# paramhanji/sin-inn

Hardware: AMD Instinct MI355X
Metric: training frames/sec at 256x256 bs=16 (higher is better)
Workload: dtype f32; 1 GPU; BASELINE configs[1]: 8-block INN (SRF, -c 4 x 2 levels), 256x256x3, fp32, synthetic clip (64 frames, lr_window 10), batch 16/GPU, full training step (fwd+bwd, rev+bwd, Adam); height=256, width=256, global_batch=16, num_coupling=4, architecture=SRF, parallelism=dp1, hip_graph=False

## Files before the change

### include/sininn.h

```cpp
#ifndef SININN_H
#define SININN_H

#include <stddef.h>
#include <stdint.h>

#ifdef __cplusplus
extern "C" {
#endif

#define SININN_ABI_VERSION 4
#define SININN_HIDDEN 256

int sininn_version(void);
const char* sininn_last_error(void);
size_t sininn_sizeof(int which);
int sininn_stream_priority_range(int* least, int* greatest);
int sininn_stream_create(int priority, void** stream);
int sininn_capture_unjoined(void* origin, void** streams, int n, int* flags);

int sininn_pack_conv_weights(const float* w_oihw, const float* bias, int N, int Cin, int ksize,
                             const int* colmap, int Np, float* w_fwd, float* b_fwd,
                             int Cdp, float* w_dgrad, void* stream);

int sininn_pack_conv_weights_bf16(const float* w_oihw, const float* bias, int N, int Cin, int ksize,
// ... 65 lines not shown
int sininn_conv_sub1_fwd(const sininn_conv_args* first, const sininn_conv_args* second, void* stream);

size_t sininn_conv_sub1_bwd_workspace_bytes(int cin, int co);
int sininn_conv_sub1_bwd(const sininn_conv_args* recompute, const sininn_conv_args* d2, const sininn_conv_args* d1, int no_dx,
                         float* gw2, float* gb2, float* gw1, float* gb1, void* workspace, size_t workspace_bytes, void* stream);

size_t sininn_conv_sub1_wide_bwd_workspace_bytes(int cin, int co);
int sininn_conv_sub1_wide_bwd(const sininn_conv_args* d2, const sininn_conv_args* d1, const float* x, int x_stride, float* gw1, float* gb1,
                              void* workspace, size_t workspace_bytes, void* stream);
size_t sininn_conv_sub1_wide_wg2_workspace_bytes(int cin, int co);
int sininn_conv_sub1_wide_wg2(const float* dr, int dr_stride, const void* h, int h_stride, int B, int H, int W, float* gw2, float* gb2,
                              void* workspace, size_t workspace_bytes, void* stream);

int sininn_conv3_smallk_bits_supported(const sininn_conv_args* args);
int sininn_conv3_smallk_bits(const sininn_conv_args* args, unsigned* bits, void* stream);

int sininn_conv_sub3_supported(const sininn_conv_args* first, const sininn_conv_args* second);
int sininn_conv_sub3(const sininn_conv_args* first, const sininn_conv_args* second, void* stream);

size_t sininn_wgrad_workspace_bytes(int N, int Cin, int ksize, int B, int H, int W);
int sininn_wgrad(const float* in, int in_stride, int Cin, const float* dout, int dout_stride, int N,
                 int B, int H, int W, int ksize, float* gw_oihw, float* gbias,
                 void* workspace, size_t workspace_bytes, void* stream);

typedef struct sininn_wgrad_item {
  size_t struct_bytes;
  const float* in;   int in_stride;   int Cin;
  const float* dout; int dout_stride; int N;
  float* gw; float* gb;
  int in_bf16, dout_bf16;
  int in_group_stride, dout_group_stride;
  int gap_begin, gap_len;
} sininn_wgrad_item;
size_t sininn_wgrad_group_workspace_bytes(const sininn_wgrad_item* items, int n, int B, int H, int W, int ksize);
int sininn_wgrad_group(const sininn_wgrad_item* items, int n, int B, int H, int W, int ksize,
                       void* workspace, size_t workspace_bytes, void* stream);

int sininn_coupling_bwd(const float* dy, int dy_stride, const int* dy_map,
                        const float* vy, int vy_stride, const int* vy_map,
                        const float* s, const float* gld, int B, int HW, int Co, float clamp,
                        int inverse, float* dr, float* dv, int dv_stride, void* stream);

int sininn_haar(const float* in, const int64_t in_strides[4], float* out, const int64_t out_strides[4],
                int B, int C, int H, int W, int inverse, void* stream);
int sininn_lrelu_bwd(float* g, int g_stride, const float* f, int f_stride, int64_t M, int n, float slope, void* stream);
int sininn_irn_tail(const float* v, int v_stride, const float* h, const float* g, int64_t M, int Co, float clamp, int inverse,
// ... 281 lines not shown
```

### sin-inn_amd/_lib.py

```python
import ctypes as C
import os

_HERE = os.path.dirname(os.path.abspath(__file__))
LIB_PATH = os.environ.get('SININN_LIB', os.path.join(_HERE, 'libsininn.so'))

c_f = C.c_void_p
c_i = C.c_void_p
I64x4 = C.c_int64 * 4


class ConvArgs(C.Structure):
    _fields_ = [
        ('inp', c_f), ('in_stride', C.c_int), ('Cin', C.c_int),
        ('w', c_f), ('bias', c_f), ('Np', C.c_int), ('winograd', C.c_int),
        ('B', C.c_int), ('H', C.c_int), ('W', C.c_int), ('ksize', C.c_int),
        ('mode', C.c_int),
        ('out', c_f), ('out_stride', C.c_int), ('N', C.c_int),
        ('out_map', c_i),
        ('v', c_f), ('v_stride', C.c_int),
        ('out2', c_f), ('out2_stride', C.c_int),
        ('sbuf', c_f),
        ('logdet', c_f),
        ('Co', C.c_int), ('clamp', C.c_float), ('col_tile', C.c_int),
        ('mask', c_f), ('mask_stride', C.c_int),
# ... 149 lines not shown
                                               C.c_void_p, C.c_void_p]),
    'sininn_pack_winograd': (C.c_int, [c_f, C.c_int, C.c_int, c_i, C.c_int, c_f, C.c_int, c_f, C.c_void_p]),
    'sininn_pack_work_items': (C.c_int, [C.POINTER(PackDesc)]),
    'sininn_pack_batch': (C.c_int, [C.c_void_p, C.c_int, C.c_int, C.c_void_p]),
    'sininn_softsplat': (C.c_int, [c_f, c_f, C.c_int, C.c_int, C.c_int, C.c_int, c_f, C.c_void_p]),
    'sininn_softsplat_bwd': (C.c_int, [c_f, c_f, c_f, C.c_int, C.c_int, C.c_int, C.c_int, c_f, c_f, C.c_void_p]),
    'sininn_occlusion_wang': (C.c_int, [c_f, C.c_int, C.c_int, C.c_int, C.c_float, c_f, c_f, C.c_void_p]),
    'sininn_census': (C.c_int, [c_f, c_f, c_f, C.c_int, C.c_int, C.c_int, C.c_int, C.c_int, C.c_float, c_f, c_f, C.c_void_p]),
    'sininn_census_bwd': (C.c_int, [c_f, c_f, c_f, C.c_int, C.c_int, C.c_int, C.c_int, C.c_int, C.c_float, c_f, c_f, c_f, c_f, C.c_void_p]),
    'sininn_masked_l1': (C.c_int, [c_f, c_f, c_f, C.c_int, C.c_int, C.c_int, C.c_int, C.c_int, C.c_float, c_f, c_f, C.c_void_p]),
    'sininn_masked_l1_bwd': (C.c_int, [c_f, c_f, c_f, C.c_int, C.c_int, C.c_int, C.c_int, C.c_int, C.c_float, c_f, c_f, c_f, c_f, C.c_void_p]),
    'sininn_occlusion_brox': (C.c_int, [c_f, c_f, C.c_int, C.c_int, C.c_int, C.c_void_p, C.c_void_p]),
    'sininn_ssim': (C.c_int, [c_f, c_f, c_f, C.c_int, C.c_int, C.c_int, C.c_int, C.c_int, C.c_int, C.c_float, c_f, c_f, C.c_void_p]),
    'sininn_ssim_bwd': (C.c_int, [c_f, c_f, c_f, C.c_int, C.c_int, C.c_int, C.c_int, C.c_int, C.c_int, C.c_float, c_f, c_f, c_f, c_f, C.c_void_p]),
    'sininn_bilateral_smooth': (C.c_int, [c_f, c_f, C.c_int, C.c_int, C.c_int, C.c_int, C.c_int, C.c_int, C.c_float, C.c_float, c_f, c_f, C.c_void_p]),
    'sininn_bilateral_smooth_bwd': (C.c_int, [c_f, c_f, C.c_int, C.c_int, C.c_int, C.c_int, C.c_int, C.c_int, C.c_float, C.c_float, c_f, c_f, C.c_void_p]),
    'sininn_coupling_colmap': (None, [C.c_int, C.c_int, C.POINTER(C.c_int)]),
    'sininn_conv': (C.c_int, [C.POINTER(ConvArgs), C.c_void_p]),
    'sininn_conv_test_hooks': (None, [C.c_int, C.c_int]),
    'sininn_wgrad_test_hooks': (None, [C.c_int]),
    'sininn_pair_k1_test_hook': (None, [C.c_int]),
    'sininn_sub1_bwd_test_hook': (None, [C.c_int]),
    'sininn_wgrad_workspace_bytes': (C.c_size_t, [C.c_int] * 6),
    'sininn_wgrad': (C.c_int, [c_f, C.c_int, C.c_int, c_f, C.c_int, C.c_int, C.c_int, C.c_int, C.c_int, C.c_int,
                               c_f, c_f, C.c_void_p, C.c_size_t, C.c_void_p]),
    'sininn_wgrad_group_workspace_bytes': (C.c_size_t, [C.POINTER(WgradItem), C.c_int, C.c_int, C.c_int, C.c_int, C.c_int]),
    'sininn_wgrad_group': (C.c_int, [C.POINTER(WgradItem), C.c_int, C.c_int, C.c_int, C.c_int, C.c_int, C.c_void_p,
                                     C.c_size_t, C.c_void_p]),
    'sininn_coupling_bwd': (C.c_int, [c_f, C.c_int, c_i, c_f, C.c_int, c_i, c_f, c_f, C.c_int, C.c_int, C.c_int,
                                      C.c_float, C.c_int, c_f, c_f, C.c_int, C.c_void_p]),
    'sininn_profile_begin': (None, [C.c_int, C.c_void_p, C.c_int]),
    'sininn_wall_clock_khz': (C.c_int, []),
    'sininn_profile_end': (C.c_int, [C.POINTER(C.c_int), C.POINTER(C.c_float)]),
    'sininn_profile_classes_begin': (None, []),
    'sininn_profile_classes_end': (C.c_int, [C.c_int, C.POINTER(C.c_double), C.POINTER(C.c_double), C.POINTER(C.c_int)]),
    'sininn_profile_classes_bytes': (C.c_int, [C.c_int, C.POINTER(C.c_double)]),
    'sininn_glow_saved_floats': (C.c_size_t, [C.c_int] * 4),
    'sininn_glow_saved_floats_dtype': (C.c_size_t, [C.c_int] * 5),
    'sininn_glow_scratch_bytes': (C.c_size_t, [C.c_int] * 5),
    'sininn_glow_scratch_bytes_dtype': (C.c_size_t, [C.c_int] * 6),
    'sininn_glow_forward': (C.c_int, [C.POINTER(GlowArgs), C.c_void_p]),
    'sininn_glow_backward': (C.c_int, [C.POINTER(GlowArgs), C.c_void_p, C.c_void_p]),
    'sininn_glow_hidden_gates': (C.c_int, [C.POINTER(GlowArgs), C.c_int, C.c_void_p, C.c_void_p]),
    'sininn_glow_group_major_fits': (C.c_int, [C.c_int, C.c_int, C.c_int]),
    'sininn_capture_unjoined': (C.c_int, [C.c_void_p, C.POINTER(C.c_void_p), C.c_int, C.POINTER(C.c_int)]),
    'sininn_conv_pair_k1_supported': (C.c_int, [C.POINTER(ConvArgs), C.POINTER(ConvArgs)]),
# ... 124 lines not shown
```

### sin-inn_amd/csrc/api.cpp

```cpp
#include <stdarg.h>
#include <string.h>

#include <unordered_map>
#include <unordered_set>
#include <vector>

#include "common.h"

namespace sininn {

static thread_local char g_err[512] = "";
void set_error(const char* fmt, ...) {
  va_list ap;
  va_start(ap, fmt);
  vsnprintf(g_err, sizeof(g_err), fmt, ap);
  va_end(ap);
}

int conv_launch(const sininn_conv_args* a, hipStream_t st);
int conv_pair_k1_supported(const sininn_conv_args* f, const sininn_conv_args* s);
size_t conv_sub1_bwd_workspace_bytes(int cond_cin, int co);
int conv_sub1_bwd_launch(const sininn_conv_args* rc, const sininn_conv_args* d2, const sininn_conv_args* d1, int no_dx, void* ws,
                         size_t ws_bytes, int* slabs_out, hipStream_t st);
int conv_sub1_bwd_reduce(int cond_cin, int co, const void* ws, int slabs, float* gw2, float* gb2, float* gw1, float* gb1, hipStream_t st);
void conv_sub1_bwd_enable(int on);
void conv3_smallk_enable(int on);
size_t conv_sub1_bf16_wide_ws_bytes(int ksize, int dtype, int cond_cin, int co);
int conv_sub1_bf16_wide_bwd_supported(const sininn_conv_args* d2, const sininn_conv_args* d1);
int conv_sub1_bf16_wide_bwd_launch(const sininn_conv_args* d2, const sininn_conv_args* d1, hipStream_t st);
int conv_sub1_bf16_wide_bwd_wg1_launch(const sininn_conv_args* d2, const sininn_conv_args* d1, const float* x, int x_stride, void* ws, size_t ws_bytes,
                                       int* slabs_out, hipStream_t st);
int conv_sub1_bf16_wide_reduce(const void* ws, int slabs, float* gw1, float* gb1, hipStream_t st);
size_t conv_sub1_bf16_wide_wg2_ws_bytes(int ksize, int dtype, int cond_cin, int co);
int conv_sub1_bf16_wide_wg2_launch(const float* dr, int dr_stride, const void* h, int h_stride, int B, int H, int W, void* ws, size_t ws_bytes,
                                   float* gw2, float* gb2, hipStream_t st);
int conv3_smallk_bf16_supported(const sininn_conv_args* a);
int conv3_smallk_bf16_launch_bits(const sininn_conv_args* a, unsigned* bits, hipStream_t st);
int conv_sub1_fwd_supported(const sininn_conv_args* f, const sininn_conv_args* s);
int conv_sub1_fwd_launch(const sininn_conv_args* f, const sininn_conv_args* s, hipStream_t st);
int conv_pair_k1_launch(const sininn_conv_args* f, const sininn_conv_args* s, hipStream_t st);
void conv_pair_k1_enable(int on);
int conv_sub3_bf16_supported(const sininn_conv_args* f, const sininn_conv_args* s);
int conv_sub3_bf16_launch(const sininn_conv_args* f, const sininn_conv_args* s, hipStream_t st);
void sub3_fusion_set(int on);
void conv_set_test_hooks(int force_cfg, int force_ck);
void wgrad_set_force16(int on);
size_t wgrad_workspace_bytes(int N, int Cin, int ksize, int B, int H, int W);
int wgrad_launch(const float* in, int in_stride, int Cin, const float* dout, int dout_stride, int N, int B, int H, int W,
                 int ksize, float* gw, float* gb, void* ws, size_t ws_bytes, hipStream_t st);
size_t wgrad_group_workspace_bytes(const sininn_wgrad_item* items, int n, int B, int H, int W, int ksize);
int wgrad_group_launch(const sininn_wgrad_item* items, int n, int B, int H, int W, int ksize, void* ws, size_t ws_bytes,
                       hipStream_t st);
int pack_launch(const float* w, const float* bias, int N, int Cin, int ksize, const int* colmap, int Np, float* w_fwd,
                float* b_fwd, int Cdp, float* w_dgrad, hipStream_t st);
int coupling_bwd_launch(const float* dy, int dy_stride, const int* dy_map, const float* vy, int vy_stride,
                        const int* vy_map, const float* s, const float* gld, int B, int HW, int Co, float clamp,
                        int inverse, float* dr, float* dv, int dv_stride, hipStream_t st);
int squeeze_launch(const float* in, const int64_t is[4], float* out, const int64_t os[4], int B, int C, int H, int W,
                   int levels, int inverse, const int* chan_map, int map_on_out, hipStream_t st);
int permute_launch(const float* in, int in_stride, float* out, int out_stride, int64_t M, int C, const int* idx,
                   hipStream_t st);
int sqdiff_sum_launch(const float* x, const int64_t xs[4], const float* y, const int64_t ys[4], int B, int C, int H,
                      int W, float* out, hipStream_t st);
int sqdiff_bwd_launch(const float* x, const int64_t xs[4], const float* y, const int64_t ys[4], int B, int C, int H,
                      int W, const float* scale, float gscale, float* gx, const int64_t gxs[4], float* gy,
                      const int64_t gys[4], hipStream_t st);
int mmd_gram_launch(const float* x, const int64_t xs[4], const float* y, const int64_t ys[4], int B, int C, int H,
                    int W, float* g, hipStream_t st);
int mmd_finish_launch(const float* g, int B, int rev, float* out, float* coef, hipStream_t st);
// ... 304 lines not shown
    SININN_CHECK(!gw1 && !gb1, "sininn_conv_sub1_wide_bwd: gw1 / gb1 need x");
    return conv_sub1_bf16_wide_bwd_launch(d2, d1, ST(stream));
  }
  int slabs = 0;
  if (int rc = conv_sub1_bf16_wide_bwd_wg1_launch(d2, d1, x, x_stride, workspace, workspace_bytes, &slabs, ST(stream))) return rc;
  if (!gw1 && !gb1) return 0;
  return conv_sub1_bf16_wide_reduce(workspace, slabs, gw1, gb1, ST(stream));
}
size_t sininn_conv_sub1_wide_wg2_workspace_bytes(int cin, int co) { return conv_sub1_bf16_wide_wg2_ws_bytes(1, 1, cin, co); }
int sininn_conv_sub1_wide_wg2(const float* dr, int dr_stride, const void* h, int h_stride, int B, int H, int W, float* gw2, float* gb2,
                              void* workspace, size_t workspace_bytes, void* stream) {
  SININN_CHECK(sininn_conv_sub1_wide_wg2_workspace_bytes(96, 96) > 0, "sininn_conv_sub1_wide_wg2: the wide kernels are switched off");
  return conv_sub1_bf16_wide_wg2_launch(dr, dr_stride, h, h_stride, B, H, W, workspace, workspace_bytes, gw2, gb2, ST(stream));
}
int sininn_conv3_smallk_bits_supported(const sininn_conv_args* args) { return conv3_smallk_bf16_supported(args); }
int sininn_conv3_smallk_bits(const sininn_conv_args* args, unsigned* bits, void* stream) {
  SININN_CHECK(bits != nullptr, "sininn_conv3_smallk_bits: bits is NULL");
  return conv3_smallk_bf16_launch_bits(args, bits, ST(stream));
}
void sininn_sub1_bwd_test_hook(int on) { conv_sub1_bwd_enable(on); conv3_smallk_enable(on); }

void sininn_conv_test_hooks(int force_cfg, int force_ck) { conv_set_test_hooks(force_cfg, force_ck); }
void sininn_wgrad_test_hooks(int force16) { wgrad_set_force16(force16); }
void sininn_pair_k1_test_hook(int on) { conv_pair_k1_enable(on & 1); sub3_fusion_set((on & 4) ? 1 : ((on & 2) ? 0 : -1)); }
int sininn_conv_sub3_supported(const sininn_conv_args* first, const sininn_conv_args* second) {
  return conv_sub3_bf16_supported(first, second);
}
int sininn_conv_sub3(const sininn_conv_args* first, const sininn_conv_args* second, void* stream) {
  return conv_sub3_bf16_launch(first, second, ST(stream));
}

size_t sininn_wgrad_workspace_bytes(int N, int Cin, int ksize, int B, int H, int W) {
  return wgrad_workspace_bytes(N, Cin, ksize, B, H, W);
}
int sininn_wgrad(const float* in, int in_stride, int Cin, const float* dout, int dout_stride, int N, int B, int H, int W,
                 int ksize, float* gw_oihw, float* gbias, void* workspace, size_t workspace_bytes, void* stream) {
  return wgrad_launch(in, in_stride, Cin, dout, dout_stride, N, B, H, W, ksize, gw_oihw, gbias, workspace,
                      workspace_bytes, ST(stream));
}

int sininn_coupling_bwd(const float* dy, int dy_stride, const int* dy_map, const float* vy, int vy_stride,
                        const int* vy_map, const float* s, const float* gld, int B, int HW, int Co, float clamp,
                        int inverse, float* dr, float* dv, int dv_stride, void* stream) {
  return coupling_bwd_launch(dy, dy_stride, dy_map, vy, vy_stride, vy_map, s, gld, B, HW, Co, clamp, inverse, dr, dv,
                             dv_stride, ST(stream));
}
// ... 243 lines not shown
```

### sin-inn_amd/csrc/glow_exec.cpp

```cpp
#include <stdlib.h>
#include <mutex>
#include <utility>
#include <vector>

#include <cstdlib>
#include "common.h"

namespace sininn {

int conv_launch(const sininn_conv_args* a, hipStream_t st);
int conv_pair_k1_supported(const sininn_conv_args* f, const sininn_conv_args* s);
int conv_pair_k1_launch(const sininn_conv_args* f, const sininn_conv_args* s, hipStream_t st);
int conv_pair_k1_preferred(const sininn_conv_args* f);
int conv_sub3_bf16_supported(const sininn_conv_args* f, const sininn_conv_args* s);
int conv_sub3_bf16_launch(const sininn_conv_args* f, const sininn_conv_args* s, hipStream_t st);
bool sub3_fusion_enabled();
size_t wgrad_workspace_bytes(int N, int Cin, int ksize, int B, int H, int W);
int wgrad_launch(const float* in, int in_stride, int Cin, const float* dout, int dout_stride, int N, int B, int H, int W,
                 int ksize, float* gw, float* gb, void* ws, size_t ws_bytes, hipStream_t st);
size_t wgrad_group_workspace_bytes(const sininn_wgrad_item* items, int n, int B, int H, int W, int ksize);
int wgrad_group_launch(const sininn_wgrad_item* items, int n, int B, int H, int W, int ksize, void* ws, size_t ws_bytes,
                       hipStream_t st);
bool wgrad_grouping_enabled();
int wgrad_group_mode();
int coupling_bwd_launch(const float* dy, int dy_stride, const int* dy_map, const float* vy, int vy_stride,
                        const int* vy_map, const float* s, const float* gld, int B, int HW, int Co, float clamp,
                        int inverse, float* dr, float* dv, int dv_stride, hipStream_t st);

static inline size_t align64(size_t n) { return (n + 63) & ~(size_t)63; }
static inline int pad16i(int n) { return (n + 15) / 16 * 16; }

static std::mutex g_ev_mutex;
struct EventRing { hipEvent_t ev[64]; bool ready = false; unsigned next = 0; };
static EventRing g_rings[16];

int conv_sub1_bwd_shape_supported(int ksize, int dtype, int cond_cin, int co);
size_t conv_sub1_bwd_workspace_bytes(int cond_cin, int co);
int conv_sub1_bwd_launch(const sininn_conv_args* rc, const sininn_conv_args* d2, const sininn_conv_args* d1, int no_dx, void* ws,
                         size_t ws_bytes, int* slabs_out, hipStream_t st);
int conv_sub1_bwd_reduce(int cond_cin, int co, const void* ws, int slabs, float* gw2, float* gb2, float* gw1, float* gb1, hipStream_t st);
int conv_sub1_fwd_supported(const sininn_conv_args* f, const sininn_conv_args* s);
int conv_sub1_fwd_launch(const sininn_conv_args* f, const sininn_conv_args* s, hipStream_t st);
size_t conv_sub1_bf16_wide_ws_bytes(int ksize, int dtype, int cond_cin, int co);
int conv_sub1_bf16_wide_bwd_supported(const sininn_conv_args* d2, const sininn_conv_args* d1);
int conv_sub1_bf16_wide_bwd_wg1_launch(const sininn_conv_args* d2, const sininn_conv_args* d1, const float* x, int x_stride, void* ws, size_t ws_bytes,
                                       int* slabs_out, hipStream_t st);
int conv_sub1_bf16_wide_reduce(const void* ws, int slabs, float* gw1, float* gb1, hipStream_t st);
// ... 205 lines not shown
                           wgrad_workspace_bytes(2 * co_a, SININN_HIDDEN, ksize, B, H, W),
                           wgrad_workspace_bytes(SININN_HIDDEN, cond_a, ksize, B, H, W)};
  for (size_t c : cands) w = c > w ? c : w;
  {
    const int cond_b = co_a;
    sininn_wgrad_item it[4] = {wgrad_item_init(), wgrad_item_init(), wgrad_item_init(), wgrad_item_init()};
    it[0].Cin = SININN_HIDDEN; it[0].N = 2 * co_b;
    it[1].Cin = cond_b;        it[1].N = SININN_HIDDEN;
    it[2].Cin = SININN_HIDDEN; it[2].N = 2 * co_a;
    it[3].Cin = cond_a;        it[3].N = SININN_HIDDEN;
    for (int pass = 0; pass < 2; ++pass) {
      if (pass == 1) {
        it[0].in_bf16 = it[2].in_bf16 = 1; it[1].dout_bf16 = it[3].dout_bf16 = 1;
      }
      for (int mask = 1; mask < 16; ++mask) {
        sininn_wgrad_item sub[4];
        int n = 0;
        for (int i = 0; i < 4; ++i)
          if (mask & (1 << i)) sub[n++] = it[i];
        const size_t bytes = wgrad_group_workspace_bytes(sub, n, B, H, W, ksize);
        w = bytes > w ? bytes : w;
      }
    }
  }
  s.ws = base + o;
  s.ws_bytes = w;
  size_t so = (o * sizeof(float) + w + 255) / 256 * 256;
  const int cond_cin[2] = {C - co_a, co_a}, cos[2] = {co_a, co_b};
  for (int i = 0; i < 2; ++i) {
    s.slab_bytes[i] = conv_sub1_bwd_shape_supported(ksize, dtype, cond_cin[i], cos[i]) ? conv_sub1_bwd_workspace_bytes(cond_cin[i], cos[i]) : 0;
    const size_t wide = conv_sub1_bf16_wide_ws_bytes(ksize, dtype, cond_cin[i], cos[i]);
    if (wide > s.slab_bytes[i]) s.slab_bytes[i] = wide;
    s.slab[i] = reinterpret_cast<char*>(base) + so;
    so += (s.slab_bytes[i] + 255) / 256 * 256;
    s.slab2_bytes[i] = conv_sub1_bf16_wide_wg2_ws_bytes(ksize, dtype, cond_cin[i], cos[i]);
    s.slab2[i] = reinterpret_cast<char*>(base) + so;
    so += (s.slab2_bytes[i] + 255) / 256 * 256;
  }
  s.total_bytes = so;
  return s;
}

size_t glow_scratch_bytes(int B, int H, int W, int C, int ksize, int dtype) {
  const int big = C - C / 2;
  Scratch s = scratch_layout(nullptr, B, H, W, C, ksize, big, big, dtype);
  return s.total_bytes + 256;
// ... 173 lines not shown
  struct Fuse { const float* vy; int vy_stride; const float* s; float* dr; };
  auto half_bwd = [&](const Half& h, const float* hbuf, const float* sbuf, float* dr, float* dh,
                      const float* dy, int dy_stride, const int* dy_map, const float* vy, int vy_stride, const int* vy_map,
                      const float* cond, int cond_stride, int cond_cin,
                      const float* addend, int add_stride, const int* add_map, float* dcond, int dcond_stride,
                      bool do_coupling, const Fuse* fuse, bool skip_d1, bool last_half) -> int {
    const sininn_subnet* net = h.net;
    if (do_coupling) {
      ClassScope sc(PC_CBWD, 3, 0.0, st);
      if (int rc = coupling_bwd_launch(dy, dy_stride, dy_map, vy, vy_stride, vy_map, sbuf, a->gld, B, HW, h.co, a->clamp, inv,
                                       dr, a->dx + h.base, C, st)) return rc;
    }
    const bool gm = group_major_hidden(a, net);
    const int gs = gm ? (int)(M * 8) : 0;
    const bool fused = fused_sub1(a, cond_cin, h.co);
    const int which_half = (&h == &hv[0]) ? 0 : 1;
    const bool wide_wg2 = bf16 && k == 1 && sc.slab2_bytes[which_half] > 0;
    if (net->gw2 && !fused && wide_wg2) {
      if (int rc = order_after(wst, st)) return rc;
      ClassScope scp(PC_WGRAD, k, conv_flops(M, k, SININN_HIDDEN, 2 * h.co), wst,
                     4.0 * (double)M * 2 * h.co + 2.0 * (double)M * SININN_HIDDEN + 2.0 * 256.0 * (2 * h.co + 1) * SININN_HIDDEN * 4.0);
      if (int rc = conv_sub1_bf16_wide_wg2_launch(dr, 2 * h.co, hbuf, SININN_HIDDEN, B, H, W, sc.slab2[which_half], sc.slab2_bytes[which_half],
                                                  net->gw2, net->gb2, wst)) return rc;
    } else if (net->gw2 && !fused) {
      if (grouped) add_item(hbuf, SININN_HIDDEN, SININN_HIDDEN, dr, 2 * h.co, 2 * h.co, net->gw2, net->gb2, bf16 ? 1 : 0, 0, gs, 0);
      else {
        if (int rc = order_after(wst, st)) return rc;
        ClassScope scp(PC_WGRAD, k, conv_flops(M, k, SININN_HIDDEN, 2 * h.co), wst);
        if (int rc = wgrad_launch(hbuf, SININN_HIDDEN, SININN_HIDDEN, dr, 2 * h.co, 2 * h.co, B, H, W, k, net->gw2, net->gb2,
                                  sc.ws, sc.ws_bytes, wst)) return rc;
      }
    }
    sininn_conv_args d2 = {};
    d2.in = dr; d2.in_stride = 2 * h.co; d2.Cin = 2 * h.co; d2.w = net->w2_dgrad; d2.Np = SININN_HIDDEN;
    d2.winograd = (net->winograd & 8) && k == 3;
    d2.B = B; d2.H = H; d2.W = W; d2.ksize = k; d2.mode = SININN_CONV_MASK;
    d2.out = dh; d2.out_stride = SININN_HIDDEN; d2.N = SININN_HIDDEN; d2.mask = hbuf; d2.mask_stride = SININN_HIDDEN;
    if (bf16) { d2.winograd = 0; d2.w_bf16 = 1; d2.in_bf16 = 0; d2.out_bf16 = 1; d2.mask_bf16 = 1; }
    if (gm) { d2.out_group_stride = gs; d2.mask_group_stride = gs; }
    sininn_conv_args d1 = {};
    d1.in = dh; d1.in_stride = SININN_HIDDEN; d1.Cin = SININN_HIDDEN; d1.w = net->w1_dgrad;
    d1.winograd = (net->winograd & 4) && k == 3;
    if (bf16) { d1.winograd = 0; d1.w_bf16 = 1; d1.in_bf16 = 1; }
    if (gm) { d1.in_stride = 8; d1.in_group_stride = gs; }
    d1.Np = d1.winograd ? (cond_cin + 31) / 32 * 32 : pad16i(cond_cin);
    d1.B = B; d1.H = H; d1.W = W; d1.ksize = k; d1.mode = SININN_CONV_ADD;
// ... 40 lines not shown
                         4.0 * (double)M * (2 * h.co + cond_cin + epi) + 2.0 * (double)M * SININN_HIDDEN);
          if (int rc_ = conv_sub1_bf16_wide_bwd_wg1_launch(&d2w, &d1, cond, cond_stride, sc.slab[which], sc.slab_bytes[which], &slabs, st)) return rc_;
        }
        if (int rc_ = order_after(wst, st)) return rc_;
        ClassScope scp(PC_WGRAD, k, 0.0, wst, (double)slabs * (cond_cin + 1) * SININN_HIDDEN * 4.0);
        return conv_sub1_bf16_wide_reduce(sc.slab[which], slabs, net->gw1, net->gb1, wst);
      }
    }
    const bool pair = !skip_d1 && conv_pair_k1_supported(&d2, &d1);
    if (pair) {
      ClassScope scp(PC_DGRAD2, k, conv_flops(M, k, 2 * h.co, SININN_HIDDEN) + conv_flops(M, k, SININN_HIDDEN, cond_cin), st);
      if (int rc = conv_pair_k1_launch(&d2, &d1, st)) return rc;
    } else {
      ClassScope scp(PC_DGRAD2, k, conv_flops(M, k, 2 * h.co, SININN_HIDDEN), st);
      sininn_conv_args f1 = {};
      f1.in = cond; f1.in_stride = cond_stride; f1.Cin = cond_cin; f1.w = net->w1; f1.bias = net->b1; f1.Np = SININN_HIDDEN;
      f1.B = B; f1.H = H; f1.W = W; f1.ksize = k; f1.mode = SININN_CONV_RELU;
      f1.out = const_cast<float*>(hbuf); f1.out_stride = SININN_HIDDEN; f1.N = SININN_HIDDEN; f1.w_bf16 = 1; f1.out_bf16 = 1;
      if (bf16 && k == 3 && conv3_smallk_bf16_supported(&f1) && conv3_smallk_bf16_supported(&d2)) {
        if (int rc = conv3_smallk_bf16_launch_bits(&d2, which_half == 0 ? sv.bits_a : sv.bits_b, st)) return rc;
      } else if (int rc = conv_launch(&d2, st)) return rc;
    }
    if (net->gw1) {
      if (grouped) add_item(cond, cond_stride, cond_cin, dh, SININN_HIDDEN, SININN_HIDDEN, net->gw1, net->gb1, 0, bf16 ? 1 : 0, 0, gs);
      else {
        if (int rc = order_after(wst, st)) return rc;
        ClassScope scp(PC_WGRAD, k, conv_flops(M, k, cond_cin, SININN_HIDDEN), wst);
        if (int rc = wgrad_launch(cond, cond_stride, cond_cin, dh, SININN_HIDDEN, SININN_HIDDEN, B, H, W, k, net->gw1, net->gb1,
                                  sc.ws, sc.ws_bytes, wst)) return rc;
      }
      if (grouped && (last_half || per_half) && n_items > 0) {
        if (int rc = order_after(wst, st)) return rc;
        double fl = 0.0;
        for (int i = 0; i < n_items; ++i) fl += conv_flops(M, k, items[i].Cin, items[i].N);
        ClassScope scp(PC_WGRAD, k, fl, wst);
        if (int rc = wgrad_group_launch(items, n_items, B, H, W, k, sc.ws, sc.ws_bytes, wst)) return rc;
        n_items = 0;
      }
    }
    if (skip_d1 || pair) return 0;
    ClassScope scp(PC_DGRAD1, k, conv_flops(M, k, SININN_HIDDEN, cond_cin), st);
    return conv_launch(&d1, st);
  };

  {
    const float* dy = a->dst_map ? a->dout : a->dout + base_b;
    const float* vy; int vy_stride; const int* vy_map = nullptr;
// ... 32 lines not shown
```

### sin-inn_amd/csrc/wgrad_mfma.hip

```cpp
#include <stdlib.h>

#include "common.h"

namespace sininn {

struct WgradDev {
  const float* in; int in_stride; int Cin;
  const float* dout; int dout_stride; int N;
  int B, H, W;
  int tiles_x, tiles_y, ntiles, tiles_per_split;
  float* partial;
  float* bpartial;
  int Nr, Cc;
  size_t in_gs, dout_gs;
  int in_bf16, dout_bf16;
};

typedef __bf16 wg_bf16x4 __attribute__((ext_vector_type(4)));
__device__ __forceinline__ f32x4 wg_load4(const float* base, size_t off, int is_bf16) {
  if (is_bf16) {
    const wg_bf16x4 v = *reinterpret_cast<const wg_bf16x4*>(reinterpret_cast<const __bf16*>(base) + off);
    return (f32x4){(float)v[0], (float)v[1], (float)v[2], (float)v[3]};
  }
  return *reinterpret_cast<const f32x4*>(base + off);
// ... 627 lines not shown
    const int cl2 = e / (4 * TAPS), r = e - cl2 * 4 * TAPS;
    const int j = r / TAPS, t2 = r - j * TAPS;
    const int col2 = lb * RC + cl2;
    if (col2 < ncol) {
      const int n = col2 / c4n, c = (col2 - n * c4n) * 4 + j;
      if (n < d.N && c < d.Cin && !(c >= q.gap_begin && c < q.gap_begin + q.gap_len)) {
        const int cw = c < q.gap_begin ? c : c - q.gap_len;
        q.gw[((size_t)n * (d.Cin - q.gap_len) + cw) * TAPS + t2] += tile[e];
      }
    }
  }
}

struct WgradPlan { int RT, CT, Nr, Cc, nblk, cblk, S, tiles_per_split, ntiles, tiles_x, tiles_y; size_t bytes; bool use32; bool wino; int th; int kh; };

void wgrad_set_bf16_mfma(int on);
static bool g_wgrad_force16 = false;
static bool g_wgrad_wino = true;
static bool g_wgrad_wino_th8 = false;
static bool g_wgrad_wino_kh2 = false;
void wgrad_set_wide_c(int on);
static int g_wgrad_group_mode = 1;
static bool g_wgrad_grouped = true;
void wgrad_set_force16(int on) { g_wgrad_force16 = (on & 1) != 0; g_wgrad_wino = (on & 2) == 0; g_wgrad_wino_th8 = (on & 4) != 0; g_wgrad_wino_kh2 = (on & 8) != 0; g_wgrad_grouped = (on & 16) == 0; g_wgrad_group_mode = (on & 32) ? 2 : 1; wgrad_set_bf16_mfma((on & 64) == 0); wgrad_set_wide_c((on & 128) == 0); }
bool wgrad_grouping_enabled() { return g_wgrad_grouped && g_wgrad_wino && !g_wgrad_force16; }
int wgrad_group_mode() { return g_wgrad_group_mode; }

static WgradPlan make_plan(int N, int Cin, int ksize, int B, int H, int W) {
  WgradPlan pl;
  pl.wino = (ksize == 3) && g_wgrad_wino;
  pl.use32 = (N % 32 == 0) && !g_wgrad_force16 && !pl.wino;
  if (N % 64 != 0 && N % 48 == 0) { pl.RT = 3; pl.CT = 4; }
  else { pl.RT = 4; pl.CT = (Cin >= 64 && ksize == 1) ? 4 : 2; }
  if (pl.use32) { pl.RT = 2; pl.CT = 2; }
  if (pl.wino) { pl.RT = 4; pl.CT = 2; }
  const int bnw = pl.RT * 16, bcw = pl.CT * 16;
  pl.nblk = (N + bnw - 1) / bnw;
  pl.cblk = (Cin + bcw - 1) / bcw;
  pl.Nr = pl.nblk * bnw;
  pl.Cc = pl.cblk * bcw;
  pl.tiles_x = (W + 15) / 16;
  pl.kh = (pl.wino && g_wgrad_wino_kh2) ? 2 : 1;
  pl.th = (pl.wino && !g_wgrad_wino_th8 && pl.kh == 1) ? 4 : WG_TH;
  pl.tiles_y = (H + pl.th - 1) / pl.th;
  pl.ntiles = B * pl.tiles_x * pl.tiles_y;
  int S = (((pl.RT == 3 && !pl.wino) || pl.kh == 2) ? 256 : 512) / (pl.nblk * pl.cblk);
  if (S < 1) S = 1;
// ... 32 lines not shown
  const WgradPlan pl = make_plan(N, Cin, ksize, B, H, W);
  SININN_CHECK(ws_bytes >= pl.bytes, "wgrad: workspace too small (%zu < %zu)", ws_bytes, pl.bytes);
  WgradDev d;
  d.in = in; d.in_stride = in_stride; d.Cin = Cin; d.dout = dout; d.dout_stride = dout_stride; d.N = N;
  d.B = B; d.H = H; d.W = W; d.tiles_x = pl.tiles_x; d.tiles_y = pl.tiles_y; d.ntiles = pl.ntiles;
  d.tiles_per_split = pl.tiles_per_split; d.Nr = pl.Nr; d.Cc = pl.Cc;
  d.in_bf16 = 0; d.dout_bf16 = 0; d.in_gs = 0; d.dout_gs = 0;
  const int taps = ksize * ksize;
  d.partial = static_cast<float*>(ws);
  d.bpartial = d.partial + (size_t)pl.S * taps * pl.Nr * pl.Cc;
  if (pl.wino) {
    if (pl.kh == 2) hipLaunchKernelGGL((wgrad_wino_kernel<8, 2, 2>), dim3(pl.S, pl.nblk, pl.cblk), dim3(512), 0, st, d);
    else if (pl.th == 4) hipLaunchKernelGGL((wgrad_wino_kernel<4, 2, 1>), dim3(pl.S, pl.nblk, pl.cblk), dim3(256), 0, st, d);
    else hipLaunchKernelGGL((wgrad_wino_kernel<8, 1, 1>), dim3(pl.S, pl.nblk, pl.cblk), dim3(256), 0, st, d);
    SININN_LAUNCH_CHECK("wgrad_wino");
  } else {
    if (ksize == 3) launch_wgrad<3>(pl, d, st); else launch_wgrad<1>(pl, d, st);
    SININN_LAUNCH_CHECK("wgrad_mfma");
  }
  const int total4 = taps * pl.Nr * (pl.Cc / 4);
  const int bias_blocks = gb ? (N + 63) / 64 : 0;
  hipLaunchKernelGGL(wgrad_reduce_kernel, dim3((total4 + 63) / 64 + bias_blocks), dim3(256), 0, st,
                     d.partial, d.bpartial, pl.S, taps, pl.Nr, pl.Cc, N, Cin, gw, gb);
  SININN_LAUNCH_CHECK("wgrad_reduce");
  return 0;
}

typedef __bf16 wgb_bf16x8 __attribute__((ext_vector_type(8)));
typedef unsigned wgb_u32x4 __attribute__((ext_vector_type(4)));

__device__ __forceinline__ unsigned pack_bf16_pair(float lo, float hi) {
  typedef __bf16 bf2 __attribute__((ext_vector_type(2)));
  bf2 v = {(__bf16)lo, (__bf16)hi};
  return *reinterpret_cast<unsigned*>(&v);
}

#ifndef WGB_ABL
#define WGB_ABL 0
#endif
#ifndef WGB_COALESCE
#define WGB_COALESCE 1
#endif
#if WGB_COALESCE
#define WGB_SLOT(f) (((f) >> 2) & 63)
#define WGB_GROUP(f) ((((f) >> 8) << 2) | ((f) & 3))
#else
// ... 442 lines not shown
```

Before: 1959 frames/s.

## Add wide-tile fp32 MFMA wgrad kernel for 1x1 coupling convs

Adds a dedicated weight-gradient kernel for 1x1 convolutions in fp32. It uses 32x32x2 f32 MFMA with multi-tile (3x2 or 2x3) register accumulators, buffer loads, double-buffered operand sets and split-K over pixels followed by the existing reduce kernel. The coupling backward routes the hidden->output and cond->hidden wgrads through it, outside the grouped wgrad path, and the workspace is sized for it. The aim is to raise per-block data reuse and MFMA throughput for these GEMM-shaped reductions, at the cost of extra workspace for partials and a separate launch per conv instead of grouping.

```diff
diff --git a/include/sininn.h b/include/sininn.h
--- a/include/sininn.h
+++ b/include/sininn.h
@@ -111,6 +111,8 @@
 int sininn_wgrad(const float* in, int in_stride, int Cin, const float* dout, int dout_stride, int N,
                  int B, int H, int W, int ksize, float* gw_oihw, float* gbias,
                  void* workspace, size_t workspace_bytes, void* stream);
+int sininn_wgrad_k1_wide_supported(int N, int Cin, int in_stride, int dout_stride, int ksize, int B, int H, int W);
+size_t sininn_wgrad_k1_wide_workspace_bytes(int N, int Cin, int in_stride, int dout_stride, int ksize, int B, int H, int W);
 
 typedef struct sininn_wgrad_item {
   size_t struct_bytes;
diff --git a/sin-inn_amd/_lib.py b/sin-inn_amd/_lib.py
--- a/sin-inn_amd/_lib.py
+++ b/sin-inn_amd/_lib.py
@@ -195,6 +195,8 @@
     'sininn_pair_k1_test_hook': (None, [C.c_int]),
     'sininn_sub1_bwd_test_hook': (None, [C.c_int]),
     'sininn_wgrad_workspace_bytes': (C.c_size_t, [C.c_int] * 6),
+    'sininn_wgrad_k1_wide_supported': (C.c_int, [C.c_int] * 8),
+    'sininn_wgrad_k1_wide_workspace_bytes': (C.c_size_t, [C.c_int] * 8),
     'sininn_wgrad': (C.c_int, [c_f, C.c_int, C.c_int, c_f, C.c_int, C.c_int, C.c_int, C.c_int, C.c_int, C.c_int,
                                c_f, c_f, C.c_void_p, C.c_size_t, C.c_void_p]),
     'sininn_wgrad_group_workspace_bytes': (C.c_size_t, [C.POINTER(WgradItem), C.c_int, C.c_int, C.c_int, C.c_int, C.c_int]),
diff --git a/sin-inn_amd/csrc/api.cpp b/sin-inn_amd/csrc/api.cpp
--- a/sin-inn_amd/csrc/api.cpp
+++ b/sin-inn_amd/csrc/api.cpp
@@ -45,6 +45,8 @@
 void sub3_fusion_set(int on);
 void conv_set_test_hooks(int force_cfg, int force_ck);
 void wgrad_set_force16(int on);
+int wgrad_k1_wide_supported(int N, int Cin, int in_stride, int dout_stride, int ksize, int B, int H, int W);
+size_t wgrad_k1_wide_workspace_bytes(int N, int Cin, int in_stride, int dout_stride, int ksize, int B, int H, int W);
 size_t wgrad_workspace_bytes(int N, int Cin, int ksize, int B, int H, int W);
 int wgrad_launch(const float* in, int in_stride, int Cin, const float* dout, int dout_stride, int N, int B, int H, int W,
                  int ksize, float* gw, float* gb, void* ws, size_t ws_bytes, hipStream_t st);
@@ -395,6 +397,12 @@
 
 void sininn_conv_test_hooks(int force_cfg, int force_ck) { conv_set_test_hooks(force_cfg, force_ck); }
 void sininn_wgrad_test_hooks(int force16) { wgrad_set_force16(force16); }
+int sininn_wgrad_k1_wide_supported(int N, int Cin, int in_stride, int dout_stride, int ksize, int B, int H, int W) {
+  return wgrad_k1_wide_supported(N, Cin, in_stride, dout_stride, ksize, B, H, W);
+}
+size_t sininn_wgrad_k1_wide_workspace_bytes(int N, int Cin, int in_stride, int dout_stride, int ksize, int B, int H, int W) {
+  return wgrad_k1_wide_workspace_bytes(N, Cin, in_stride, dout_stride, ksize, B, H, W);
+}
 void sininn_pair_k1_test_hook(int on) { conv_pair_k1_enable(on & 1); sub3_fusion_set((on & 4) ? 1 : ((on & 2) ? 0 : -1)); }
 int sininn_conv_sub3_supported(const sininn_conv_args* first, const sininn_conv_args* second) {
   return conv_sub3_bf16_supported(first, second);
diff --git a/sin-inn_amd/csrc/glow_exec.cpp b/sin-inn_amd/csrc/glow_exec.cpp
--- a/sin-inn_amd/csrc/glow_exec.cpp
+++ b/sin-inn_amd/csrc/glow_exec.cpp
@@ -23,6 +23,10 @@
                        hipStream_t st);
 bool wgrad_grouping_enabled();
 int wgrad_group_mode();
+int wgrad_k1_wide_supported(int N, int Cin, int in_stride, int dout_stride, int ksize, int B, int H, int W);
+size_t wgrad_k1_wide_workspace_bytes(int N, int Cin, int in_stride, int dout_stride, int ksize, int B, int H, int W);
+int wgrad_k1_wide_launch(const float* in, int in_stride, int Cin, const float* dout, int dout_stride, int N, int B, int H, int W,
+                         float* gw, float* gb, void* ws, size_t ws_bytes, hipStream_t st);
 int coupling_bwd_launch(const float* dy, int dy_stride, const int* dy_map, const float* vy, int vy_stride,
                         const int* vy_map, const float* s, const float* gld, int B, int HW, int Co, float clamp,
                         int inverse, float* dr, float* dv, int dv_stride, hipStream_t st);
@@ -274,6 +278,14 @@
         w = bytes > w ? bytes : w;
       }
     }
+  }
+  if (dtype == 0 && ksize == 1) {
+    const int cond_b = co_a;
+    const size_t wide[4] = {wgrad_k1_wide_workspace_bytes(2 * co_b, SININN_HIDDEN, SININN_HIDDEN, 2 * co_b, ksize, B, H, W),
+                            wgrad_k1_wide_workspace_bytes(SININN_HIDDEN, cond_b, C, SININN_HIDDEN, ksize, B, H, W),
+                            wgrad_k1_wide_workspace_bytes(2 * co_a, SININN_HIDDEN, SININN_HIDDEN, 2 * co_a, ksize, B, H, W),
+                            wgrad_k1_wide_workspace_bytes(SININN_HIDDEN, cond_a, C, SININN_HIDDEN, ksize, B, H, W)};
+    for (size_t c : wide) w = c > w ? c : w;
   }
   s.ws = base + o;
   s.ws_bytes = w;
@@ -493,6 +505,14 @@
                      4.0 * (double)M * 2 * h.co + 2.0 * (double)M * SININN_HIDDEN + 2.0 * 256.0 * (2 * h.co + 1) * SININN_HIDDEN * 4.0);
       if (int rc = conv_sub1_bf16_wide_wg2_launch(dr, 2 * h.co, hbuf, SININN_HIDDEN, B, H, W, sc.slab2[which_half], sc.slab2_bytes[which_half],
                                                   net->gw2, net->gb2, wst)) return rc;
+    } else if (net->gw2 && !fused && !bf16 && wgrad_k1_wide_supported(2 * h.co, SININN_HIDDEN, SININN_HIDDEN, 2 * h.co, k, B, H, W) &&
+               sc.ws_bytes >= wgrad_k1_wide_workspace_bytes(2 * h.co, SININN_HIDDEN, SININN_HIDDEN, 2 * h.co, k, B, H, W)) {
+      if (int rc = order_after(wst, st)) return rc;
+      const double slabs = (double)wgrad_k1_wide_workspace_bytes(2 * h.co, SININN_HIDDEN, SININN_HIDDEN, 2 * h.co, k, B, H, W);
+      ClassScope scp(PC_WGRAD, k, conv_flops(M, k, SININN_HIDDEN, 2 * h.co), wst,
+                     4.0 * (double)M * (2 * h.co + SININN_HIDDEN) + 2.0 * slabs);
+      if (int rc = wgrad_k1_wide_launch(hbuf, SININN_HIDDEN, SININN_HIDDEN, dr, 2 * h.co, 2 * h.co, B, H, W, net->gw2, net->gb2,
+                                        sc.ws, sc.ws_bytes, wst)) return rc;
     } else if (net->gw2 && !fused) {
       if (grouped) add_item(hbuf, SININN_HIDDEN, SININN_HIDDEN, dr, 2 * h.co, 2 * h.co, net->gw2, net->gb2, bf16 ? 1 : 0, 0, gs, 0);
       else {
@@ -579,7 +599,15 @@
       } else if (int rc = conv_launch(&d2, st)) return rc;
     }
     if (net->gw1) {
-      if (grouped) add_item(cond, cond_stride, cond_cin, dh, SININN_HIDDEN, SININN_HIDDEN, net->gw1, net->gb1, 0, bf16 ? 1 : 0, 0, gs);
+      if (!bf16 && wgrad_k1_wide_supported(SININN_HIDDEN, cond_cin, cond_stride, SININN_HIDDEN, k, B, H, W) &&
+          sc.ws_bytes >= wgrad_k1_wide_workspace_bytes(SININN_HIDDEN, cond_cin, cond_stride, SININN_HIDDEN, k, B, H, W)) {
+        if (int rc = order_after(wst, st)) return rc;
+        const double slabs = (double)wgrad_k1_wide_workspace_bytes(SININN_HIDDEN, cond_cin, cond_stride, SININN_HIDDEN, k, B, H, W);
+        ClassScope scp(PC_WGRAD, k, conv_flops(M, k, cond_cin, SININN_HIDDEN), wst,
+                       4.0 * (double)M * (cond_cin + SININN_HIDDEN) + 2.0 * slabs);
+        if (int rc = wgrad_k1_wide_launch(cond, cond_stride, cond_cin, dh, SININN_HIDDEN, SININN_HIDDEN, B, H, W, net->gw1, net->gb1,
+                                          sc.ws, sc.ws_bytes, wst)) return rc;
+      } else if (grouped) add_item(cond, cond_stride, cond_cin, dh, SININN_HIDDEN, SININN_HIDDEN, net->gw1, net->gb1, 0, bf16 ? 1 : 0, 0, gs);
       else {
         if (int rc = order_after(wst, st)) return rc;
         ClassScope scp(PC_WGRAD, k, conv_flops(M, k, cond_cin, SININN_HIDDEN), wst);
diff --git a/sin-inn_amd/csrc/wgrad_mfma.hip b/sin-inn_amd/csrc/wgrad_mfma.hip
--- a/sin-inn_amd/csrc/wgrad_mfma.hip
+++ b/sin-inn_amd/csrc/wgrad_mfma.hip
@@ -673,7 +673,9 @@
 void wgrad_set_wide_c(int on);
 static int g_wgrad_group_mode = 1;
 static bool g_wgrad_grouped = true;
-void wgrad_set_force16(int on) { g_wgrad_force16 = (on & 1) != 0; g_wgrad_wino = (on & 2) == 0; g_wgrad_wino_th8 = (on & 4) != 0; g_wgrad_wino_kh2 = (on & 8) != 0; g_wgrad_grouped = (on & 16) == 0; g_wgrad_group_mode = (on & 32) ? 2 : 1; wgrad_set_bf16_mfma((on & 64) == 0); wgrad_set_wide_c((on & 128) == 0); }
+static bool g_wgrad_k1_wide = true;
+static bool g_wgrad_k1_wide_c1 = true;
+void wgrad_set_force16(int on) { g_wgrad_force16 = (on & 1) != 0; g_wgrad_wino = (on & 2) == 0; g_wgrad_wino_th8 = (on & 4) != 0; g_wgrad_wino_kh2 = (on & 8) != 0; g_wgrad_grouped = (on & 16) == 0; g_wgrad_group_mode = (on & 32) ? 2 : 1; wgrad_set_bf16_mfma((on & 64) == 0); wgrad_set_wide_c((on & 128) == 0); g_wgrad_k1_wide = (on & 256) == 0; g_wgrad_k1_wide_c1 = (on & 512) == 0; }
 bool wgrad_grouping_enabled() { return g_wgrad_grouped && g_wgrad_wino && !g_wgrad_force16; }
 int wgrad_group_mode() { return g_wgrad_group_mode; }
 
@@ -752,6 +754,177 @@
   const int bias_blocks = gb ? (N + 63) / 64 : 0;
   hipLaunchKernelGGL(wgrad_reduce_kernel, dim3((total4 + 63) / 64 + bias_blocks), dim3(256), 0, st,
                      d.partial, d.bpartial, pl.S, taps, pl.Nr, pl.Cc, N, Cin, gw, gb);
+  SININN_LAUNCH_CHECK("wgrad_reduce");
+  return 0;
+}
+
+constexpr int WGK1_D = 8;
+constexpr int WGK1_PIX = 8 * WGK1_D;
+struct WgK1Dev {
+  const float* in; const float* dout;
+  unsigned in_stride, dout_stride, in_bytes, dout_bytes;
+  int N, Cin, pps;
+  float* partial;
+  float* bpartial;
+};
+
+template <int NW>
+__device__ __forceinline__ void wgk1_load(__amdgpu_buffer_rsrc_t rs, unsigned off, float (&dst)[NW]) {
+  static_assert(NW == 2 || NW == 3, "8- or 12-byte operand loads");
+  if constexpr (NW == 2) {
+    const auto v = __builtin_amdgcn_raw_buffer_load_b64(rs, (int)off, 0, 0);
+    dst[0] = __uint_as_float(v[0]); dst[1] = __uint_as_float(v[1]);
+  } else {
+    const auto v = __builtin_amdgcn_raw_buffer_load_b96(rs, (int)off, 0, 0);
+    dst[0] = __uint_as_float(v[0]); dst[1] = __uint_as_float(v[1]); dst[2] = __uint_as_float(v[2]);
+  }
+}
+
+template <int NA, int NB>
+__global__ __launch_bounds__(256, 2) void wgrad_k1_wide_kernel(WgK1Dev p) {
+  __shared__ __attribute__((aligned(16))) float lds[4 * 16 * 64];
+  const int tid = threadIdx.x;
+  const int wave = tid >> 6, lane = tid & 63;
+  const int li = lane & 31, kh = lane >> 5;
+  const int split = blockIdx.x, n0 = blockIdx.y * 32 * NA, c0 = blockIdx.z * 32 * NB;
+  const __amdgpu_buffer_rsrc_t a_rs = __builtin_amdgcn_make_buffer_rsrc(const_cast<float*>(p.dout), 0, (int)p.dout_bytes, 0x00020000);
+  const __amdgpu_buffer_rsrc_t b_rs = __builtin_amdgcn_make_buffer_rsrc(const_cast<float*>(p.in), 0, (int)p.in_bytes, 0x00020000);
+  const unsigned pix = (unsigned)split * (unsigned)p.pps + 2u * wave + kh;
+  unsigned aoff = (pix * p.dout_stride + (unsigned)(n0 + NA * li)) * 4u;
+  unsigned boff = (pix * p.in_stride + (unsigned)(c0 + NB * li)) * 4u;
+  const unsigned astep = 32u * p.dout_stride, bstep = 32u * p.in_stride;
+
+  f32x16 acc[NA][NB];
+#pragma unroll
+  for (int i = 0; i < NA; ++i)
+#pragma unroll
+    for (int j = 0; j < NB; ++j)
+#pragma unroll
+      for (int q = 0; q < 16; ++q) acc[i][j][q] = 0.f;
+  float bsum[NA];
+#pragma unroll
+  for (int i = 0; i < NA; ++i) bsum[i] = 0.f;
+
+  float xa[WGK1_D][NA], xb[WGK1_D][NB], ya[WGK1_D][NA], yb[WGK1_D][NB];
+  auto load_set = [&](float (&sa)[WGK1_D][NA], float (&sb)[WGK1_D][NB], bool live) {
+#pragma unroll
+    for (int u = 0; u < WGK1_D; ++u) {
+      wgk1_load<NA>(a_rs, live ? aoff : BUF_OOB, sa[u]);
+      wgk1_load<NB>(b_rs, live ? boff : BUF_OOB, sb[u]);
+      aoff += astep; boff += bstep;
+    }
+  };
+  auto mfma_set = [&](const float (&sa)[WGK1_D][NA], const float (&sb)[WGK1_D][NB]) {
+#pragma unroll
+    for (int u = 0; u < WGK1_D; ++u)
+#pragma unroll
+      for (int i = 0; i < NA; ++i) {
+        bsum[i] += sa[u][i];
+#pragma unroll
+        for (int j = 0; j < NB; ++j) acc[i][j] = __builtin_amdgcn_mfma_f32_32x32x2f32(sa[u][i], sb[u][j], acc[i][j], 0, 0, 0);
+      }
+  };
+  const int nsteps = p.pps / 8;
+  load_set(xa, xb, true);
+  for (int s0 = 0; s0 < nsteps; s0 += 2 * WGK1_D) {
+    load_set(ya, yb, s0 + WGK1_D < nsteps);
+    __builtin_amdgcn_sched_barrier(0);
+    mfma_set(xa, xb);
+    __builtin_amdgcn_sched_barrier(0);
+    load_set(xa, xb, s0 + 2 * WGK1_D < nsteps);
+    __builtin_amdgcn_sched_barrier(0);
+    mfma_set(ya, yb);
+    __builtin_amdgcn_sched_barrier(0);
+  }
+
+#pragma unroll
+  for (int t = 0; t < NA * NB; ++t) {
+    const int i = t / NB, j = t % NB;
+#pragma unroll
+    for (int q = 0; q < 16; ++q) lds[(wave * 16 + q) * 64 + lane] = acc[i][j][q];
+    __syncthreads();
+#pragma unroll
+    for (int r = 0; r < 4; ++r) {
+      const int q = wave * 4 + r;
+      const float v = (lds[(0 * 16 + q) * 64 + lane] + lds[(1 * 16 + q) * 64 + lane]) +
+                      (lds[(2 * 16 + q) * 64 + lane] + lds[(3 * 16 + q) * 64 + lane]);
+      const int n = n0 + NA * ((q & 3) + 8 * (q >> 2) + 4 * kh) + i;
+      const int c = c0 + NB * li + j;
+      p.partial[((size_t)split * p.N + n) * p.Cin + c] = v;
+    }
+    __syncthreads();
+  }
+#pragma unroll
+  for (int i = 0; i < NA; ++i) {
+    bsum[i] += __shfl_xor(bsum[i], 32);
+    if (lane < 32) lds[(wave * NA + i) * 32 + lane] = bsum[i];
+  }
+  __syncthreads();
+  if (blockIdx.z == 0 && tid < 32) {
+#pragma unroll
+    for (int i = 0; i < NA; ++i)
+      p.bpartial[(size_t)split * p.N + n0 + NA * tid + i] =
+          (lds[(0 * NA + i) * 32 + tid] + lds[(1 * NA + i) * 32 + tid]) + (lds[(2 * NA + i) * 32 + tid] + lds[(3 * NA + i) * 32 + tid]);
+  }
+}
+
+struct WgK1Plan { int na, nb, nblk, cblk, S, pps; size_t bytes; };
+static bool wgk1_plan(int N, int Cin, int in_stride, int dout_stride, int ksize, size_t M, bool hooks, WgK1Plan& pl) {
+  if (ksize != 1 || M == 0 || N <= 0 || Cin <= 0) return false;
+  if (hooks && (!g_wgrad_k1_wide || !g_wgrad_grouped || g_wgrad_force16)) return false;
+  if (N % 96 == 0 && Cin % 64 == 0) { pl.na = 3; pl.nb = 2; }
+  else if (N % 64 == 0 && Cin % 96 == 0) { pl.na = 2; pl.nb = 3; if (hooks && !g_wgrad_k1_wide_c1) return false; }
+  else return false;
+  pl.nblk = N / (32 * pl.na);
+  pl.cblk = Cin / (32 * pl.nb);
+  if (pl.nblk * pl.cblk > 256) return false;
+  const size_t target = 256 / (size_t)(pl.nblk * pl.cblk);
+  const size_t pps = ((M + target - 1) / target + WGK1_PIX - 1) / WGK1_PIX * WGK1_PIX;
+  const size_t S = (M + pps - 1) / pps;
+  const size_t stride = (size_t)(in_stride > dout_stride ? in_stride : dout_stride);
+  if ((S * pps + WGK1_PIX) * stride * 4 >= (1ull << 31) || S > 65535) return false;
+  pl.pps = (int)pps; pl.S = (int)S;
+  pl.bytes = (S * (size_t)N * Cin + S * (size_t)N) * sizeof(float);
+  return true;
+}
+
+int wgrad_k1_wide_supported(int N, int Cin, int in_stride, int dout_stride, int ksize, int B, int H, int W) {
+  WgK1Plan pl;
+  if (B <= 0 || H <= 0 || W <= 0 || in_stride < Cin || dout_stride < N) return 0;
+  return wgk1_plan(N, Cin, in_stride, dout_stride, ksize, (size_t)B * H * W, true, pl) ? 1 : 0;
+}
+
+size_t wgrad_k1_wide_workspace_bytes(int N, int Cin, int in_stride, int dout_stride, int ksize, int B, int H, int W) {
+  WgK1Plan pl;
+  if (B <= 0 || H <= 0 || W <= 0 || in_stride < Cin || dout_stride < N) return 0;
+  return wgk1_plan(N, Cin, in_stride, dout_stride, ksize, (size_t)B * H * W, false, pl) ? pl.bytes : 0;
+}
+
+int wgrad_k1_wide_launch(const float* in, int in_stride, int Cin, const float* dout, int dout_stride, int N,
+                         int B, int H, int W, float* gw, float* gb, void* ws, size_t ws_bytes, hipStream_t st) {
+  SININN_CHECK(in && dout && gw && ws, "wgrad_k1_wide: null pointer");
+  SININN_CHECK(B > 0 && H > 0 && W > 0 && in_stride >= Cin && dout_stride >= N, "wgrad_k1_wide: bad shape");
+  SININN_CHECK((reinterpret_cast<uintptr_t>(in) & 3) == 0 && (reinterpret_cast<uintptr_t>(dout) & 3) == 0 && aligned16(ws),
+               "wgrad_k1_wide: misaligned pointer");
+  const size_t M = (size_t)B * H * W;
+  WgK1Plan pl;
+  SININN_CHECK(wgk1_plan(N, Cin, in_stride, dout_stride, 1, M, false, pl), "wgrad_k1_wide: unsupported problem N=%d Cin=%d (check wgrad_k1_wide_supported first)", N, Cin);
+  SININN_CHECK(ws_bytes >= pl.bytes, "wgrad_k1_wide: workspace too small (%zu < %zu)", ws_bytes, pl.bytes);
+  WgK1Dev d;
+  d.in = in; d.dout = dout; d.in_stride = (unsigned)in_stride; d.dout_stride = (unsigned)dout_stride;
+  d.in_bytes = (unsigned)(((M - 1) * in_stride + Cin) * 4);
+  d.dout_bytes = (unsigned)(((M - 1) * dout_stride + N) * 4);
+  d.N = N; d.Cin = Cin; d.pps = pl.pps;
+  d.partial = static_cast<float*>(ws);
+  d.bpartial = d.partial + (size_t)pl.S * N * Cin;
+  const dim3 grid(pl.S, pl.nblk, pl.cblk);
+  if (pl.na == 3) hipLaunchKernelGGL((wgrad_k1_wide_kernel<3, 2>), grid, dim3(256), 0, st, d);
+  else hipLaunchKernelGGL((wgrad_k1_wide_kernel<2, 3>), grid, dim3(256), 0, st, d);
+  SININN_LAUNCH_CHECK("wgrad_k1_wide");
+  const int total4 = N * (Cin / 4);
+  const int bias_blocks = gb ? (N + 63) / 64 : 0;
+  hipLaunchKernelGGL(wgrad_reduce_kernel, dim3((total4 + 63) / 64 + bias_blocks), dim3(256), 0, st,
+                     d.partial, d.bpartial, pl.S, 1, N, Cin, N, Cin, gw, gb);
   SININN_LAUNCH_CHECK("wgrad_reduce");
   return 0;
 }
```

After: 1967 frames/s, median of 6. No clear change (+0.4%).
